# radiocosmology/draco

Hardware: AMD Instinct MI355X
Metric: m-modes/sec through MModeTransform+DirtyMapMaker (128-feed, 256-freq) (higher is better)
Workload: dtype f64 accumulate; B stored complex128; FFT complex64 (as the reference); 1 GPU; cfg3: 128-feed (379 stacked baselines), 256 freq per GPU (256 in the job), 1024 RA, lmax=mmax=512: MModeTransform.process + DirtyMapMaker.process through the task classes (131328 (m,f) solves + alm2map to nside=256 IQUV maps per GPU and day); parallelism=freq-sharded x1, weak scaling (no collective in the timed region)

## Files before the change

### draco_amd/csrc/sht.hip

```cpp
#include "sht_common.h"
#include "sht_legendre.h"
#include "sht_rings.h"

namespace {

int get_geom(dmm_ctx* ctx, int nside, int lmax, int mmax, ShtGeom* out) {
  const int64_t key = ((int64_t)nside << 40) | ((int64_t)lmax << 20) | (int64_t)mmax;
  auto it = ctx->sht.find(key);
  const int nring = 4 * nside - 1;
  const size_t nd = (size_t)3 * nring + (mmax + 1);
  const size_t bytes = nd * sizeof(double) + (size_t)nring * sizeof(int64_t) + (size_t)nring * sizeof(int);
  const size_t coef_ofs = (bytes + 63) / 64 * 64;
  const size_t coef_rows = (size_t)coef_row0(mmax + 1, lmax);
  int blue_rmax = 0;
  std::vector<int64_t> bf_off(1, 0);
  int64_t bf_total = 0;
  for (int ir = 1; ir < nside && blue_len(ir) <= kMaxBlue; ++ir) {
    bf_off.push_back(bf_total);
    bf_total += blue_len(ir);
    blue_rmax = ir;
  }
  const size_t bfo_ofs = coef_ofs + coef_rows * sizeof(Coef);
  const size_t bf_ofs = (bfo_ofs + bf_off.size() * sizeof(int64_t) + 63) / 64 * 64;
  const size_t phase_ofs = (bf_ofs + (size_t)bf_total * sizeof(double2) + 63) / 64 * 64;
  int tw_len = kMaxBlue;
  while (tw_len < 4 * nside) tw_len <<= 1;
  const size_t tw_ofs = phase_ofs + (size_t)nring * (mmax + 1) * sizeof(double2);
  const size_t chirp_ofs = tw_ofs + (size_t)(tw_len / 2) * sizeof(double2);
  const size_t total = chirp_ofs + (size_t)2 * blue_rmax * (blue_rmax + 1) * sizeof(double2);
  if (it == ctx->sht.end()) {
    std::vector<unsigned char> h(bytes);
    double* z = reinterpret_cast<double*>(h.data());
    double* sth = z + nring;
    double* phi0 = sth + nring;
    double* lfac = phi0 + nring;
    int64_t* start = reinterpret_cast<int64_t*>(lfac + (mmax + 1));
    int* nphi = reinterpret_cast<int*>(start + nring);
    const int64_t npix = 12LL * nside * nside, ncap = 2LL * nside * (nside - 1);
    for (int k = 0; k < nring; ++k) {
      const int64_t ir = k + 1;
      if (ir < nside) {
        z[k] = 1.0 - (double)(ir * ir) / (3.0 * nside * (double)nside);
        nphi[k] = (int)(4 * ir);
        phi0[k] = M_PI / (4.0 * ir);
        start[k] = 2 * ir * (ir - 1);
      } else if (ir <= 3LL * nside) {
        z[k] = (2.0 * nside - ir) * 2.0 / (3.0 * nside);
        nphi[k] = 4 * nside;
        phi0[k] = ((ir - nside + 1) & 1) * M_PI / (4.0 * nside);
        start[k] = ncap + (ir - nside) * 4LL * nside;
      } else {
        const int64_t ip = 4LL * nside - ir;
        z[k] = -(1.0 - (double)(ip * ip) / (3.0 * nside * (double)nside));
        nphi[k] = (int)(4 * ip);
        phi0[k] = M_PI / (4.0 * ip);
        start[k] = npix - 2 * ip * (ip + 1);
      }
      sth[k] = sqrt((1.0 - z[k]) * (1.0 + z[k]));
    }
    double acc = 0.5 * (log2(1.0) - log2(4.0 * M_PI));
    lfac[0] = acc;
    double prod = 0.0;
    for (int m = 1; m <= mmax; ++m) {
      prod += log2((2.0 * m - 1.0) / (2.0 * m));
      lfac[m] = 0.5 * (log2(2.0 * m + 1.0) - log2(4.0 * M_PI) + prod);
    }
    void* d = nullptr;
    DMM_HIP(hipMalloc(&d, total));
    unsigned char* db = static_cast<unsigned char*>(d);
    hipError_t e = hipMemcpy(d, h.data(), bytes, hipMemcpyHostToDevice);
    if (e == hipSuccess) e = hipMemcpy(db + bfo_ofs, bf_off.data(), bf_off.size() * sizeof(int64_t), hipMemcpyHostToDevice);
    if (e == hipSuccess) {
      hipLaunchKernelGGL(k_fill_coef, dim3(mmax + 1), dim3(256), 0, ctx->stream, reinterpret_cast<Coef*>(db + coef_ofs), lmax);
      e = hipGetLastError();
    }
    if (e == hipSuccess && blue_rmax > 0) {
      const int Mmax = blue_len(blue_rmax);
      const size_t lds = ((size_t)Mmax + 1 + Mmax / 2) * sizeof(double2);
      e = hipFuncSetAttribute((const void*)k_build_bfilt, hipFuncAttributeMaxDynamicSharedMemorySize, (int)lds);
      if (e == hipSuccess) {
        hipLaunchKernelGGL(k_build_bfilt, dim3(blue_rmax), dim3(kFftThreads), lds, ctx->stream,
                           reinterpret_cast<double2*>(db + bf_ofs), reinterpret_cast<const int64_t*>(db + bfo_ofs));
        e = hipGetLastError();
      }
    }
    if (e == hipSuccess) {
      hipLaunchKernelGGL(k_fill_ring_tables, dim3(nring + 1 + blue_rmax), dim3(256), 0, ctx->stream,
                         reinterpret_cast<const double*>(db) + 2 * (size_t)nring , nring, mmax,
                         reinterpret_cast<double2*>(db + phase_ofs), reinterpret_cast<double2*>(db + tw_ofs), tw_len,
                         reinterpret_cast<double2*>(db + chirp_ofs));
      e = hipGetLastError();
    }
    if (e != hipSuccess) {
      (void)hipFree(d);
      return dmm_set_error((int)e, "sht geometry upload: %s", hipGetErrorString(e));
    }
    it = ctx->sht.emplace(key, d).first;
  }
  ShtGeom g;
  g.nside = nside;
  g.lmax = lmax;
  g.mmax = mmax;
  g.nring = nring;
  g.block = it->second;
  g.z = reinterpret_cast<double*>(g.block);
  g.sth = g.z + nring;
  g.phi0 = g.sth + nring;
  g.lfac = g.phi0 + nring;
  g.start = reinterpret_cast<int64_t*>(g.lfac + (mmax + 1));
  g.nphi = reinterpret_cast<int*>(g.start + nring);
  unsigned char* gb = static_cast<unsigned char*>(g.block);
  g.coef = reinterpret_cast<double*>(gb + coef_ofs);
  g.bf_off = reinterpret_cast<int64_t*>(gb + bfo_ofs);
  g.bfilt = reinterpret_cast<double2*>(gb + bf_ofs);
  g.blue_rmax = blue_rmax;
  g.phase = reinterpret_cast<double2*>(gb + phase_ofs);
  g.tw = reinterpret_cast<double2*>(gb + tw_ofs);
  g.tw_len = tw_len;
  g.chirp = reinterpret_cast<double2*>(gb + chirp_ofs);
  *out = g;
  return DMM_OK;
}

int check_args(const char* who, dmm_ctx* ctx, const void* a, const void* b, int nfreq, int npol, int lmax, int mmax,
               int nside) {
  DMM_REQUIRE(ctx && a && b, "%s: NULL argument", who);
  DMM_REQUIRE(nfreq >= 1 && lmax >= 0 && mmax >= 0 && mmax <= lmax, "%s: bad sizes nfreq=%d lmax=%d mmax=%d", who, nfreq, lmax, mmax);
  DMM_REQUIRE(npol == 1 || npol == 4, "%s: npol must be 1 or 4 (got %d)", who, npol);
  DMM_REQUIRE(nside >= 1 && (nside & (nside - 1)) == 0 && nside <= 8192, "%s: nside must be a power of two (got %d)", who, nside);
  return DMM_OK;
}

size_t chunk_freqs(int nfreq, int npol, int nring, int mmax) {
  const size_t grp = npol == 4 ? kSynF : 1;
  const size_t per_f = (size_t)npol * nring * (mmax + 1) * sizeof(double2);
  size_t nf = ((size_t)1 << 30) / per_f / grp * grp;
  if (nf < grp) nf = grp;
  if (nf > (size_t)nfreq) nf = nfreq;
  const size_t nchunk = ((size_t)nfreq + nf - 1) / nf;
  const size_t c = ((size_t)nfreq + nchunk - 1) / nchunk;
  return c < (size_t)nfreq ? (c + grp - 1) / grp * grp : c;
}

size_t coef_scratch_bytes(size_t nfc, int npol, int nring, int mmax) {
  const size_t nfs = npol == 4 ? (nfc + kSynF - 1) / kSynF * kSynF : nfc;
  return nfs * npol * nring * (size_t)(mmax + 1) * sizeof(double2);
}

struct ClassLaunch {
  RingClass rc;
  int nblock;
  int nphi_max;
  bool blue;
};

std::vector<ClassLaunch> ring_classes(const ShtGeom& g) {
  std::vector<ClassLaunch> out;
  ClassLaunch b;
  b.rc.belt = 1;
  b.rc.r_lo = b.rc.r_hi = 0;
  b.rc.M = 4 * g.nside;
  b.rc.logM = 0;
  while ((1 << b.rc.logM) < b.rc.M) ++b.rc.logM;
  b.nblock = 2 * g.nside + 1;
  b.nphi_max = 4 * g.nside;
  b.blue = false;
  out.push_back(b);
  for (int ir = 1; ir < g.nside;) {
    const int M = blue_len(ir);
    int hi = ir;
    while (hi + 1 < g.nside && blue_len(hi + 1) == M) ++hi;
    ClassLaunch c;
    c.rc.belt = 0;
    c.rc.r_lo = ir;
    c.rc.r_hi = hi;
    c.rc.M = M;
    c.rc.logM = 0;
    while ((1 << c.rc.logM) < M) ++c.rc.logM;
    c.nblock = 2 * (hi - ir + 1);
    c.nphi_max = 4 * hi;
    c.blue = true;
    out.push_back(c);
    ir = hi + 1;
  }
  return out;
}

size_t ring_fft_lds(const ShtGeom& g, const ClassLaunch& c, int nrow, int force_direct) {
  if (force_direct) return 0;
  if (c.blue && c.rc.r_hi > g.blue_rmax) return 0;
  const size_t lds = ((size_t)nrow * (c.rc.M + 1) + c.rc.M / 2 + (c.blue ? c.nphi_max : 0)) * sizeof(double2);
  return lds <= 160 * 1024 ? lds : 0;
}

size_t ring_synth_lds(const ShtGeom& g, const ClassLaunch& c, int nb, bool stage_all, int force_direct) {
  if (force_direct) return 0;
  if (c.blue && c.rc.r_hi > g.blue_rmax) return 0;
  const int nm = g.mmax + 1;
  const bool staged = stage_all || 4 * (c.blue ? c.rc.r_lo : g.nside) < nm;
  const size_t lds = ((size_t)nb * (c.rc.M + 1) + c.rc.M / 2 + (c.blue ? c.nphi_max : 0) + (staged ? (size_t)nb * 2 * nm : 0)) *
                     sizeof(double2);
  return lds <= 160 * 1024 ? lds : 0;
}

template <typename K>
int launch_ring(K kern, dim3 grid, int threads, size_t lds, hipStream_t st, const RingParams& rp, const RingClass& rc) {
  if (lds > 160 * 1024) return dmm_set_error(DMM_E_UNSUPPORTED, "SHT ring stage needs %zu bytes of LDS (nside too large)", lds);
  DMM_HIP(hipFuncSetAttribute((const void*)kern, hipFuncAttributeMaxDynamicSharedMemorySize, (int)lds));
  hipLaunchKernelGGL(kern, grid, dim3(threads), lds, st, rp, rc);
  DMM_HIP(hipGetLastError());
  return DMM_OK;
}

template <int NPOL>
int synth_chunk(dmm_ctx* ctx, const ShtGeom& g, const double2* alm, int n_m, int nf, double2* b, double* map) {
  LegParams lp;
  lp.g = g;
  lp.nf = nf;
  lp.npol = NPOL;
  lp.n_m = n_m;
  lp.alm = alm;
  lp.b = b;
  if (NPOL == 4 && !(ctx->opt_sht_variant & 8)) {
    const int npair = (g.nring + 1) / 2;
    const int nrc = (npair + kThreads - 1) / kThreads;
#ifdef LEG_STAMPS
    static unsigned long long* stamps_d = nullptr;
    const size_t nst = (size_t)(g.mmax + 1) * nrc * ((nf + 2 * kLegF - 1) / (2 * kLegF)) * 4 * 8;
    if (!stamps_d) (void)hipMalloc((void**)&stamps_d, 64 << 20);
    (void)hipMemsetAsync(stamps_d, 0, nst * 8, ctx->stream);
    lp.stamps = stamps_d;
#endif
    const int nx = g.mmax + 1;
    const int64_t col_bytes = (int64_t)4 * n_m * (g.lmax + 1) * (int64_t)sizeof(double2);
    const bool fits8 = 2 * kLegF * col_bytes < ((int64_t)1 << 32), fits4 = kLegF * col_bytes < ((int64_t)1 << 32);
    if ((ctx->opt_sht_variant & 64) || ctx->opt_sht_synth_form == 1 || !fits4) {
      const int nz = (nf + kLegF - 1) / kLegF;
      hipLaunchKernelGGL(k_leg_synth_mfma, dim3(nx, nrc, nz), dim3(kThreads), 0, ctx->stream, lp);
    } else if ((ctx->opt_sht_variant & 128) || !fits8) {
      const int nz = (nf + kLegF - 1) / kLegF;
      hipLaunchKernelGGL(k_leg_synth_mfma2<1>, dim3(nx, nrc, nz), dim3(kThreads), 0, ctx->stream, lp);
    } else {
      const int nz = (nf + 2 * kLegF - 1) / (2 * kLegF);
      hipLaunchKernelGGL(k_leg_synth_mfma2<2>, dim3(nx, nrc, nz), dim3(kThreads), 0, ctx->stream, lp);
    }
  } else
  switch (ctx->opt_sht_variant & 3) {
    case 1: hipLaunchKernelGGL((k_leg_synth<NPOL, 1, 1>), dim3(g.mmax + 1, nf), dim3(kThreads), 0, ctx->stream, lp); break;
    case 2: hipLaunchKernelGGL((k_leg_synth<NPOL, 2, 1>), dim3(g.mmax + 1, nf), dim3(kThreads), 0, ctx->stream, lp); break;
    case 3: hipLaunchKernelGGL((k_leg_synth<NPOL, 1, 6>), dim3(g.mmax + 1, nf), dim3(kThreads), 0, ctx->stream, lp); break;
    default: hipLaunchKernelGGL((k_leg_synth<NPOL, 2, 4>), dim3(g.mmax + 1, nf), dim3(kThreads), 0, ctx->stream, lp); break;
  }
  DMM_HIP(hipGetLastError());
  RingParams rp;
  rp.g = g;
  rp.nf = nf;
  rp.npol = NPOL;
  rp.b = b;
  rp.map = map;
  rp.map_ref = nullptr;
  rp.radix8 = (ctx->opt_sht_variant & 2048) ? 0 : 1;
  rp.npix = 12LL * g.nside * g.nside;
  rp.stage_all = 0;
  constexpr int KF = NPOL == 4 ? kSynF : 1;
  const dim3 per_ring((nf + KF - 1) / KF, NPOL == 4 ? 2 : 1);
  const int force_direct = ctx->opt_sht_variant & 4;
  for (const ClassLaunch& c : ring_classes(g)) {
    int nb = 0;
    size_t lds = 0;
    rp.stage_all = 0;
    for (int tier = 0; tier < 3 && nb == 0; ++tier)
      for (int b = KF; b >= 1 && nb == 0; b >>= 1) {
        const size_t l = ring_synth_lds(g, c, b, tier == 0, force_direct);
        if (l != 0 && l <= (tier < 2 ? (size_t)80 * 1024 : (size_t)160 * 1024)) nb = b, lds = l, rp.stage_all = tier == 0;
      }
    const dim3 grid(c.nblock, per_ring.x, per_ring.y);
    int rc;
    if (nb == 0) {
      rc = launch_ring(k_ring_synth<NPOL>, dim3(c.nblock, nf), kThreads, (size_t)NPOL * (g.mmax + 1) * sizeof(double2), ctx->stream, rp, c.rc);
    } else if (nb == 4) {
      rc = c.blue ? launch_ring(k_ring_synth_fft<NPOL, NPOL == 4 ? 4 : 1, true>, grid, kFftThreads, lds, ctx->stream, rp, c.rc)
                  : launch_ring(k_ring_synth_fft<NPOL, NPOL == 4 ? 4 : 1, false>, grid, kFftThreads, lds, ctx->stream, rp, c.rc);
    } else if (nb == 2) {
      rc = c.blue ? launch_ring(k_ring_synth_fft<NPOL, NPOL == 4 ? 2 : 1, true>, grid, kFftThreads, lds, ctx->stream, rp, c.rc)
                  : launch_ring(k_ring_synth_fft<NPOL, NPOL == 4 ? 2 : 1, false>, grid, kFftThreads, lds, ctx->stream, rp, c.rc);
    } else {
      rc = c.blue ? launch_ring(k_ring_synth_fft<NPOL, 1, true>, grid, kFftThreads, lds, ctx->stream, rp, c.rc)
                  : launch_ring(k_ring_synth_fft<NPOL, 1, false>, grid, kFftThreads, lds, ctx->stream, rp, c.rc);
    }
    if (rc) return rc;
  }
  return DMM_OK;
}

template <int NPOL>
int anal_chunk(dmm_ctx* ctx, const ShtGeom& g, const double* map, int n_m, int nf, double2* b, double2* alm, int accumulate,
               const double* map_ref = nullptr) {
  RingParams rp;
  rp.g = g;
  rp.nf = nf;
  rp.npol = NPOL;
  rp.b = b;
  rp.map = const_cast<double*>(map);
  rp.map_ref = map_ref;
  rp.radix8 = (ctx->opt_sht_variant & 2048) ? 0 : 1;
  rp.npix = 12LL * g.nside * g.nside;
  rp.stage_all = 0;
  constexpr int NROWS = NPOL == 4 ? 2 : 1;
  const int force_direct = ctx->opt_sht_variant & 4;
  for (const ClassLaunch& c : ring_classes(g)) {
    const size_t lds2 = ring_fft_lds(g, c, NROWS, force_direct), lds1 = ring_fft_lds(g, c, 1, force_direct);
    int rc;
    if (lds1 == 0) {
      rc = launch_ring(k_ring_anal<NPOL>, dim3(c.nblock, nf), kThreads, (size_t)NPOL * c.nphi_max * sizeof(double), ctx->stream, rp, c.rc);
    } else if (NROWS == 2 && lds2 != 0 && lds2 <= 80 * 1024) {
      rc = c.blue ? launch_ring(k_ring_anal_fft<NPOL, NROWS, true>, dim3(c.nblock, nf), kFftThreads, lds2, ctx->stream, rp, c.rc)
                  : launch_ring(k_ring_anal_fft<NPOL, NROWS, false>, dim3(c.nblock, nf), kFftThreads, lds2, ctx->stream, rp, c.rc);
    } else {
      rc = c.blue ? launch_ring(k_ring_anal_fft<NPOL, 1, true>, dim3(c.nblock, nf, NROWS), kFftThreads, lds1, ctx->stream, rp, c.rc)
                  : launch_ring(k_ring_anal_fft<NPOL, 1, false>, dim3(c.nblock, nf, NROWS), kFftThreads, lds1, ctx->stream, rp, c.rc);
    }
    if (rc) return rc;
  }
  LegAnalParams lp;
  lp.g = g;
  lp.nf = nf;
  lp.npol = NPOL;
  lp.n_m = n_m;
  lp.b = b;
  lp.alm = alm;
  lp.accumulate = accumulate;
  lp.m_identity = (ctx->opt_sht_variant & 32) ? 1 : 0;
  if (NPOL == 4 && !(ctx->opt_sht_variant & 8)) {
    if (ctx->opt_sht_variant & 16)
      hipLaunchKernelGGL((k_leg_anal_mfma<kAnThreads, 1>), dim3(g.mmax + 1, (nf + kLegF - 1) / kLegF), dim3(kAnThreads), 0, ctx->stream, lp);
    else
      hipLaunchKernelGGL((k_leg_anal_mfma<256, 1>), dim3(g.mmax + 1, (nf + kLegF - 1) / kLegF), dim3(256), 0, ctx->stream, lp);
    DMM_HIP(hipGetLastError());
    return DMM_OK;
  }
  constexpr int NV = NPOL == 4 ? 8 : 2;
  const size_t lds2 = (size_t)(g.lmax + 1) * NV * sizeof(double) + (size_t)2 * (kThreads / 64) * kAnalBatch * NV * sizeof(double);
  DMM_HIP(hipFuncSetAttribute((const void*)k_leg_anal<NPOL>, hipFuncAttributeMaxDynamicSharedMemorySize, (int)lds2));
  hipLaunchKernelGGL(k_leg_anal<NPOL>, dim3(g.mmax + 1, nf), dim3(kThreads), lds2, ctx->stream, lp);
  DMM_HIP(hipGetLastError());
  return DMM_OK;
}

}

extern "C" {

int dmm_alm2map(dmm_ctx* ctx, const void* alm, int nfreq, int npol, int lmax, int mmax, int nside, double* map) {
  int rc = check_args("dmm_alm2map", ctx, alm, map, nfreq, npol, lmax, mmax, nside);
  if (rc) return rc;
  DMM_HIP(hipSetDevice(ctx->device));
  ShtGeom g;
  rc = get_geom(ctx, nside, lmax, mmax, &g);
  if (rc) return rc;
  const size_t nfc = chunk_freqs(nfreq, npol, g.nring, mmax);
  void* scratch = nullptr;
  rc = dmm_get_scratch(ctx, coef_scratch_bytes(nfc, npol, g.nring, mmax), &scratch);
  if (rc) return rc;
  const int64_t npix = 12LL * nside * nside;
  const int n_m = mmax + 1;
  for (int f0 = 0; f0 < nfreq; f0 += (int)nfc) {
    const int nf = (int)((size_t)(nfreq - f0) < nfc ? (size_t)(nfreq - f0) : nfc);
    const double2* a = (const double2*)alm + (int64_t)f0 * npol * n_m * (lmax + 1);
    double* mp = map + (int64_t)f0 * npol * npix;
    rc = npol == 4 ? synth_chunk<4>(ctx, g, a, n_m, nf, (double2*)scratch, mp) : synth_chunk<1>(ctx, g, a, n_m, nf, (double2*)scratch, mp);
    if (rc) return rc;
  }
  return DMM_OK;
}

int dmm_map2alm(dmm_ctx* ctx, const double* map, int nfreq, int npol, int lmax, int mmax, int nside, int niter,
                void* alm) {
  int rc = check_args("dmm_map2alm", ctx, map, alm, nfreq, npol, lmax, mmax, nside);
  if (rc) return rc;
  DMM_REQUIRE(niter >= 0 && niter <= 64, "dmm_map2alm: niter=%d out of range", niter);
  if ((size_t)npol * 4 * nside * sizeof(double) > 150 * 1024)
    return dmm_set_error(DMM_E_UNSUPPORTED, "dmm_map2alm: nside=%d too large for the in-LDS ring stage", nside);
  DMM_HIP(hipSetDevice(ctx->device));
  ShtGeom g;
  rc = get_geom(ctx, nside, lmax, mmax, &g);
  if (rc) return rc;
  const int64_t npix = 12LL * nside * nside;
  size_t nfc = chunk_freqs(nfreq, npol, g.nring, mmax);
  const size_t b_bytes = coef_scratch_bytes(nfc, npol, g.nring, mmax);
  const size_t r_bytes = niter > 0 ? nfc * npol * (size_t)npix * sizeof(double) : 0;
  void* scratch = nullptr;
  rc = dmm_get_scratch(ctx, b_bytes + r_bytes, &scratch);
  if (rc) return rc;
  double2* b = (double2*)scratch;
  double* resid = (double*)((unsigned char*)scratch + b_bytes);
  const int n_m = mmax + 1;
  for (int f0 = 0; f0 < nfreq; f0 += (int)nfc) {
    const int nf = (int)((size_t)(nfreq - f0) < nfc ? (size_t)(nfreq - f0) : nfc);
    double2* a = (double2*)alm + (int64_t)f0 * npol * n_m * (lmax + 1);
    const double* mp = map + (int64_t)f0 * npol * npix;
    rc = npol == 4 ? anal_chunk<4>(ctx, g, mp, n_m, nf, b, a, 0) : anal_chunk<1>(ctx, g, mp, n_m, nf, b, a, 0);
    if (rc) return rc;
    for (int it = 0; it < niter; ++it) {
      rc = npol == 4 ? synth_chunk<4>(ctx, g, a, n_m, nf, b, resid) : synth_chunk<1>(ctx, g, a, n_m, nf, b, resid);
      if (rc) return rc;
      rc = npol == 4 ? anal_chunk<4>(ctx, g, resid, n_m, nf, b, a, 1, mp) : anal_chunk<1>(ctx, g, resid, n_m, nf, b, a, 1, mp);
      if (rc) return rc;
    }
  }
  return DMM_OK;
}

}
```

### draco_amd/csrc/sht_rings.h

```cpp
#pragma once
#include "sht_common.h"

namespace {

struct RingParams {
  ShtGeom g;
  int nf, npol;
  double2* b;
  double* map;
  int64_t npix;
  const double* map_ref;
  int radix8;
  int stage_all;
};

struct RingClass {
  int belt;
  int r_lo, r_hi;
  int M, logM;
};
constexpr int kMinBlue = 256, kMaxBlue = 4096;

__host__ __device__ __forceinline__ int blue_len(int ir) {
  int M = kMinBlue;
  while (M < 8 * ir - 1) M <<= 1;
  return M;
}

__device__ __forceinline__ int class_ring(const RingClass& rc, const ShtGeom& g, int i) {
  if (rc.belt) return g.nside - 1 + i;
  const int ir = rc.r_lo + (i >> 1);
  return (i & 1) ? g.nring - ir : ir - 1;
}

template <int NPOL>
__global__ __launch_bounds__(kThreads) void k_ring_synth(RingParams p, RingClass rc) {
  extern __shared__ __align__(16) unsigned char smem[];
  double2* c = reinterpret_cast<double2*>(smem);
  const int ring = class_ring(rc, p.g, blockIdx.x);
  const int f = blockIdx.y;
  const int nm = p.g.mmax + 1;
  const double phi0 = p.g.phi0[ring];
  const int nphi = p.g.nphi[ring];
  for (int idx = threadIdx.x; idx < NPOL * nm; idx += kThreads) {
    const int pol = idx / nm, m = idx - pol * nm;
    double2 v;
    if (NPOL == 1) {
      v = p.b[((int64_t)f * p.g.nring + ring) * nm + m];
    } else {
      const double* q = reinterpret_cast<const double*>(p.b) + syn4_at(f, m, ring, pol >> 1, p.g.nring, nm) + syn4_slot(pol);
      v = make_double2(q[0], q[2]);
    }
    double sn, cs;
    sincos((double)m * phi0, &sn, &cs);
    const double fac = m == 0 ? 1.0 : 2.0;
    c[idx] = make_double2(fac * (v.x * cs - v.y * sn), fac * (v.x * sn + v.y * cs));
  }
  __syncthreads();
  const int64_t base = p.g.start[ring];
  for (int j = threadIdx.x; j < nphi; j += kThreads) {
    double sn, cs;
    sincospi(2.0 * (double)j / (double)nphi, &sn, &cs);
    double pr = 1.0, pi_ = 0.0;
    double acc[NPOL];
#pragma unroll
    for (int q = 0; q < NPOL; ++q) acc[q] = 0.0;
    for (int m = 0; m < nm; ++m) {
#pragma unroll
      for (int q = 0; q < NPOL; ++q) {
        const double2 cm = c[q * nm + m];
        acc[q] = fma(cm.x, pr, fma(-cm.y, pi_, acc[q]));
      }
      const double nr = pr * cs - pi_ * sn;
      pi_ = fma(pr, sn, pi_ * cs);
      pr = nr;
    }
#pragma unroll
    for (int q = 0; q < NPOL; ++q) p.map[((int64_t)f * NPOL + q) * p.npix + base + j] = acc[q];
  }
}

constexpr int kFftThreads = 256;

struct RingLds {
  dmm_fft::C<double>* buf;
  dmm_fft::C<double>* tw;
  dmm_fft::C<double>* chirp;
};

template <int NROW, bool BLUE>
__device__ __forceinline__ RingLds ring_lds(unsigned char* smem, const ShtGeom& g, int N, int M) {
  RingLds l;
  l.buf = reinterpret_cast<dmm_fft::C<double>*>(smem);
  l.tw = l.buf + NROW * (M + 1);
  l.chirp = l.tw + (M >> 1);
  const int stride = g.tw_len / M;
  for (int k = threadIdx.x; k < (M >> 1); k += kFftThreads) {
    const double2 t = g.tw[k * stride];
    l.tw[k] = {t.x, t.y};
  }
  if (BLUE) {
    const int ir = N >> 2;
    const double2* src = g.chirp + (int64_t)2 * ir * (ir - 1);
    for (int k = threadIdx.x; k < N; k += kFftThreads) {
      const double2 t = src[k];
      l.chirp[k] = {t.x, t.y};
    }
  }
  return l;
}

__global__ void k_fill_ring_tables(const double* phi0, int nring, int mmax, double2* phase, double2* tw, int tw_len,
                                   double2* chirp) {
  const int b = blockIdx.x;
  if (b < nring) {
    const double p0 = phi0[b];
    for (int m = threadIdx.x; m <= mmax; m += blockDim.x) {
      double sn, cs;
      sincos((double)m * p0, &sn, &cs);
      phase[(int64_t)b * (mmax + 1) + m] = make_double2(cs, sn);
    }
  } else if (b == nring) {
    for (int k = threadIdx.x; k < tw_len / 2; k += blockDim.x) {
      double sn, cs;
      sincospi(-2.0 * (double)k / (double)tw_len, &sn, &cs);
      tw[k] = make_double2(cs, sn);
    }
  } else {
    const int ir = b - nring, N = 4 * ir;
    double2* dst = chirp + (int64_t)2 * ir * (ir - 1);
    for (int k = threadIdx.x; k < N; k += blockDim.x) {
      const int k2 = (int)(((int64_t)k * k) % (2 * (int64_t)N));
      double sn, cs;
      sincospi(-(double)k2 / (double)N, &sn, &cs);
      dst[k] = make_double2(cs, sn);
    }
  }
}

template <int NROW, bool BLUE>
__device__ __forceinline__ void ring_dft(const RingLds& l, const double2* bfilt, int M, int logM, bool radix8 = false) {
  const int P = M + 1;
  if (radix8) dmm_fft::fft_dif8<double, kFftThreads>(l.buf, l.tw, NROW, M, logM, P);
  else dmm_fft::fft_dif<double, kFftThreads>(l.buf, l.tw, NROW, M, logM, P);
  if (BLUE) {
    for (int idx = threadIdx.x; idx < NROW * M; idx += kFftThreads) {
      const int r = idx / M, k = idx - r * M;
      const double2 fk = bfilt[k];
      l.buf[r * P + k] = dmm_fft::cmul<double>(l.buf[r * P + k], {fk.x, fk.y});
    }
    __syncthreads();
    if (radix8) dmm_fft::fft_dit8<double, true, kFftThreads>(l.buf, l.tw, NROW, M, logM, P);
    else dmm_fft::fft_dit<double, true, kFftThreads>(l.buf, l.tw, NROW, M, logM, P);
  }
}

template <bool BLUE>
__device__ __forceinline__ dmm_fft::C<double> ring_dft_at(const RingLds& l, int r, int k, int M, int logM) {
  if (BLUE) return dmm_fft::cmul<double>(l.buf[r * (M + 1) + k], l.chirp[k]);
  return l.buf[r * (M + 1) + dmm_fft::bitrev(k, logM)];
}

template <int NPOL, int NB, bool BLUE>
__global__ __launch_bounds__(kFftThreads) void k_ring_synth_fft(RingParams p, RingClass rc) {
  using dmm_fft::C;
  constexpr int KF = NPOL == 4 ? kSynF : 1;
  static_assert(KF % NB == 0, "passes of NB transforms");
  extern __shared__ __align__(16) unsigned char smem[];
  const int ring = class_ring(rc, p.g, blockIdx.x), r = NPOL == 4 ? (int)blockIdx.z : 0;
  const int f0 = KF * blockIdx.y, nfb = min(KF, p.nf - f0);
  const int n = p.g.nphi[ring], M = rc.M, P = M + 1;
  const RingLds l = ring_lds<NB, BLUE>(smem, p.g, n, M);
  if (BLUE) __syncthreads();
  const int nm = p.g.mmax + 1;
  const double2* phase = p.g.phase + (int64_t)ring * nm;
  auto load = [&](int fi, int m, double2& va, double2& vb) {
    if (NPOL == 1) {
      va = p.b[((int64_t)(f0 + fi) * p.g.nring + ring) * nm + m];
    } else {
      const double* q = reinterpret_cast<const double*>(p.b) + syn4_at(f0 + fi, m, ring, r, p.g.nring, nm);
      const double2 re = *reinterpret_cast<const double2*>(q), im = *reinterpret_cast<const double2*>(q + 2);
      va = r == 0 ? make_double2(re.x, im.x) : make_double2(re.y, im.y);
      vb = r == 0 ? make_double2(re.y, im.y) : make_double2(re.x, im.x);
    }
  };
  const bool staged = p.stage_all || n < nm;
  C<double>* rot = l.chirp + (BLUE ? 4 * rc.r_hi : 0);
  const double2* bfilt = BLUE ? p.g.bfilt + p.g.bf_off[rc.belt ? 0 : rc.r_lo + ((int)blockIdx.x >> 1)] : nullptr;
  const int64_t base = p.g.start[ring];
  for (int fb = 0; fb < nfb; fb += NB) {
    if (fb > 0) __syncthreads();
    if (staged) {
      for (int q = threadIdx.x; q < NB * nm; q += kFftThreads) {
        const int m = q / NB, j = q - m * NB;
        C<double> a = {0.0, 0.0}, b = {0.0, 0.0};
        if (fb + j < nfb) {
          const double2 ph = phase[m];
          const double cs = ph.x, sn = ph.y;
          double2 va, vb;
          load(fb + j, m, va, vb);
          a = {va.x * cs - va.y * sn, va.x * sn + va.y * cs};
          if (NPOL == 4) b = {vb.x * cs - vb.y * sn, vb.x * sn + vb.y * cs};
          if (m == 0) a.y = b.y = 0.0;
        }
        rot[(j * 2 + 0) * nm + m] = a;
        rot[(j * 2 + 1) * nm + m] = b;
      }
      __syncthreads();
    }
    for (int k = threadIdx.x; k < M; k += kFftThreads) {
      double zr[NB], zi[NB];
#pragma unroll
      for (int j = 0; j < NB; ++j) zr[j] = zi[j] = 0.0;
      if (k < n && staged) {
        for (int m = k; m < nm; m += n) {
#pragma unroll
          for (int j = 0; j < NB; ++j) {
            const C<double> a = rot[(j * 2 + 0) * nm + m], b = rot[(j * 2 + 1) * nm + m];
            zr[j] += a.x - b.y;
            zi[j] += a.y + b.x;
          }
        }
        for (int m = (k == 0 ? n : n - k); m < nm; m += n) {
#pragma unroll
          for (int j = 0; j < NB; ++j) {
            const C<double> a = rot[(j * 2 + 0) * nm + m], b = rot[(j * 2 + 1) * nm + m];
            zr[j] += a.x + b.y;
            zi[j] += b.x - a.y;
          }
        }
      } else if (k < n) {
        for (int m = k; m < nm; m += n) {
          const double2 ph = phase[m];
          const double cs = ph.x, sn = ph.y;
#pragma unroll
          for (int j = 0; j < NB; ++j) {
            if (fb + j >= nfb) continue;
            double2 va, vb;
            load(fb + j, m, va, vb);
            double ar = va.x * cs - va.y * sn, ai = va.x * sn + va.y * cs;
            double br = 0.0, bi = 0.0;
            if (NPOL == 4) {
              br = vb.x * cs - vb.y * sn;
              bi = vb.x * sn + vb.y * cs;
            }
            if (m == 0) ai = bi = 0.0;
            zr[j] += ar - bi;
            zi[j] += ai + br;
          }
        }
        for (int m = (k == 0 ? n : n - k); m < nm; m += n) {
          const double2 ph = phase[m];
          const double cs = ph.x, sn = ph.y;
#pragma unroll
          for (int j = 0; j < NB; ++j) {
            if (fb + j >= nfb) continue;
            double2 va, vb;
            load(fb + j, m, va, vb);
            const double ar = va.x * cs - va.y * sn, ai = va.x * sn + va.y * cs;
            double br = 0.0, bi = 0.0;
            if (NPOL == 4) {
              br = vb.x * cs - vb.y * sn;
              bi = vb.x * sn + vb.y * cs;
            }
            zr[j] += ar + bi;
            zi[j] += br - ai;
          }
        }
      }
#pragma unroll
      for (int j = 0; j < NB; ++j) {
        C<double> v = {zr[j], -zi[j]};
        if (BLUE && k < n) v = dmm_fft::cmul<double>(v, l.chirp[k]);
        l.buf[j * P + k] = v;
      }
    }
    __syncthreads();
    ring_dft<NB, BLUE>(l, bfilt, M, rc.logM, p.radix8 != 0);
    for (int j = threadIdx.x; j < n; j += kFftThreads) {
#pragma unroll
      for (int jj = 0; jj < NB; ++jj) {
        if (fb + jj >= nfb) continue;
        const int64_t f = f0 + fb + jj;
        const C<double> y = ring_dft_at<BLUE>(l, jj, j, M, rc.logM);
        p.map[(f * NPOL + 2 * r) * p.npix + base + j] = y.x;
        if (NPOL == 4) p.map[(f * NPOL + 2 * r + 1) * p.npix + base + j] = -y.y;
      }
    }
  }
}

template <int NPOL>
__global__ __launch_bounds__(kThreads) void k_ring_anal(RingParams p, RingClass rc) {
  extern __shared__ __align__(16) unsigned char smem[];
  double* px = reinterpret_cast<double*>(smem);
  const int ring = class_ring(rc, p.g, blockIdx.x), f = blockIdx.y;
  const int nm = p.g.mmax + 1;
  const double phi0 = p.g.phi0[ring];
  const int nphi = p.g.nphi[ring];
  const int64_t base = p.g.start[ring];
  for (int idx = threadIdx.x; idx < NPOL * nphi; idx += kThreads) {
    const int pol = idx / nphi, j = idx - pol * nphi;
    const int64_t pi = ((int64_t)f * NPOL + pol) * p.npix + base + j;
    px[idx] = p.map_ref ? p.map_ref[pi] - p.map[pi] : p.map[pi];
  }
  __syncthreads();
  const double w = 4.0 * M_PI / (double)p.npix;
  for (int m = threadIdx.x; m < nm; m += kThreads) {
    double sn, cs;
    sincospi(-2.0 * (double)(m % nphi) / (double)nphi, &sn, &cs);
    double pr = 1.0, pi_ = 0.0;
    double are[NPOL], aim[NPOL];
#pragma unroll
    for (int q = 0; q < NPOL; ++q) are[q] = aim[q] = 0.0;
    for (int j = 0; j < nphi; ++j) {
#pragma unroll
      for (int q = 0; q < NPOL; ++q) {
        const double v = px[q * nphi + j];
        are[q] = fma(v, pr, are[q]);
        aim[q] = fma(v, pi_, aim[q]);
      }
      const double nr = pr * cs - pi_ * sn;
      pi_ = fma(pr, sn, pi_ * cs);
      pr = nr;
    }
    double s0, c0;
    sincos(-(double)m * phi0, &s0, &c0);
#pragma unroll
    for (int q = 0; q < NPOL; ++q)
      p.b[(((int64_t)f * NPOL + q) * p.g.nring + ring) * nm + m] =
          make_double2(w * (are[q] * c0 - aim[q] * s0), w * (are[q] * s0 + aim[q] * c0));
  }
}

template <int NPOL, int NROW, bool BLUE>
__global__ __launch_bounds__(kFftThreads) void k_ring_anal_fft(RingParams p, RingClass rc) {
  using dmm_fft::C;
  extern __shared__ __align__(16) unsigned char smem[];
  const int rb = blockIdx.z * NROW;
  const int ring = class_ring(rc, p.g, blockIdx.x), f = blockIdx.y;
  const int n = p.g.nphi[ring], M = rc.M, P = M + 1;
  const RingLds l = ring_lds<NROW, BLUE>(smem, p.g, n, M);
  if (BLUE) __syncthreads();
  const int64_t base = p.g.start[ring];
  for (int k = threadIdx.x; k < M; k += kFftThreads) {
#pragma unroll
    for (int r = 0; r < NROW; ++r) {
      C<double> v = {0.0, 0.0};
      if (k < n) {
        const int64_t p0 = ((int64_t)f * NPOL + (NPOL == 4 ? 2 * (r + rb) : 0)) * p.npix + base + k, p1 = p0 + p.npix;
        v.x = p.map_ref ? p.map_ref[p0] - p.map[p0] : p.map[p0];
        if (NPOL == 4) v.y = p.map_ref ? p.map_ref[p1] - p.map[p1] : p.map[p1];
        if (BLUE) v = dmm_fft::cmul<double>(v, l.chirp[k]);
      }
      l.buf[r * P + k] = v;
    }
  }
  __syncthreads();
  const double2* bfilt = BLUE ? p.g.bfilt + p.g.bf_off[rc.belt ? 0 : rc.r_lo + ((int)blockIdx.x >> 1)] : nullptr;
  ring_dft<NROW, BLUE>(l, bfilt, M, rc.logM, p.radix8 != 0);
  const int nm = p.g.mmax + 1;
  const double2* phase = p.g.phase + (int64_t)ring * nm;
  const double w = 4.0 * M_PI / (double)p.npix;
  for (int m = threadIdx.x; m < nm; m += kFftThreads) {
    const int k = m % n, k2 = (n - k) % n;
    const double2 ph = phase[m];
    const double c0 = ph.x, s0 = -ph.y;
#pragma unroll
    for (int r = 0; r < NROW; ++r) {
      const C<double> X = ring_dft_at<BLUE>(l, r, k, M, rc.logM), Y = ring_dft_at<BLUE>(l, r, k2, M, rc.logM);
      const double ar = 0.5 * (X.x + Y.x), ai = 0.5 * (X.y - Y.y);
      p.b[(((int64_t)f * NPOL + (NPOL == 4 ? 2 * (r + rb) : 0)) * p.g.nring + ring) * nm + m] =
          make_double2(w * (ar * c0 - ai * s0), w * (ar * s0 + ai * c0));
      if (NPOL == 4) {
        const double br = 0.5 * (X.y + Y.y), bi = -0.5 * (X.x - Y.x);
        p.b[(((int64_t)f * NPOL + 2 * (r + rb) + 1) * p.g.nring + ring) * nm + m] =
            make_double2(w * (br * c0 - bi * s0), w * (br * s0 + bi * c0));
      }
    }
  }
}

__global__ __launch_bounds__(kFftThreads) void k_build_bfilt(double2* table, const int64_t* bf_off) {
  using dmm_fft::C;
  extern __shared__ __align__(16) unsigned char smem[];
  const int ir = blockIdx.x + 1, N = 4 * ir, M = blue_len(ir), P = M + 1;
  int logM = 0;
  while ((1 << logM) < M) ++logM;
  C<double>* buf = reinterpret_cast<C<double>*>(smem);
  C<double>* tw = buf + P;
  for (int k = threadIdx.x; k < (M >> 1); k += kFftThreads) {
    double sn, cs;
    sincospi(-2.0 * (double)k / (double)M, &sn, &cs);
    tw[k] = {cs, sn};
  }
  for (int j = threadIdx.x; j < M; j += kFftThreads) {
    const int nn = j < N ? j : (j > M - N ? M - j : -1);
    C<double> v = {0.0, 0.0};
    if (nn >= 0) {
      const int k2 = (int)(((int64_t)nn * nn) % (2 * (int64_t)N));
      double sn, cs;
      sincospi((double)k2 / (double)N, &sn, &cs);
      v = {cs, sn};
    }
    buf[j] = v;
  }
  __syncthreads();
  dmm_fft::fft_dif<double, kFftThreads>(buf, tw, 1, M, logM, P);
  const double inv = 1.0 / (double)M;
  double2* out = table + bf_off[ir];
  for (int k = threadIdx.x; k < M; k += kFftThreads) out[k] = make_double2(buf[k].x * inv, buf[k].y * inv);
}

}
```

Measured before the change: 2059 m-modes/s.

## Add register-accumulating synth4 ring kernel that folds m-phases before FFT

```diff
diff --git a/draco_amd/csrc/sht.hip b/draco_amd/csrc/sht.hip
--- a/draco_amd/csrc/sht.hip
+++ b/draco_amd/csrc/sht.hip
@@ -193,14 +193,35 @@
   return lds <= 160 * 1024 ? lds : 0;
 }
 
-size_t ring_synth_lds(const ShtGeom& g, const ClassLaunch& c, int nb, bool stage_all, int force_direct) {
+size_t ring_synth_lds(const ShtGeom& g, const ClassLaunch& c, bool stage_all, int force_direct) {
   if (force_direct) return 0;
   if (c.blue && c.rc.r_hi > g.blue_rmax) return 0;
   const int nm = g.mmax + 1;
   const bool staged = stage_all || 4 * (c.blue ? c.rc.r_lo : g.nside) < nm;
-  const size_t lds = ((size_t)nb * (c.rc.M + 1) + c.rc.M / 2 + (c.blue ? c.nphi_max : 0) + (staged ? (size_t)nb * 2 * nm : 0)) *
-                     sizeof(double2);
+  const size_t lds = ((size_t)(c.rc.M + 1) + c.rc.M / 2 + (c.blue ? c.nphi_max : 0) + (staged ? (size_t)2 * nm : 0)) * sizeof(double2);
   return lds <= 160 * 1024 ? lds : 0;
+}
+
+struct Synth4Shape {
+  int nrow, kt, seg;
+  size_t lds;
+};
+Synth4Shape ring_synth4_shape(const ShtGeom& g, const ClassLaunch& c, int force_direct) {
+  Synth4Shape s = {1, 0, 0, 0};
+  if (force_direct || (c.blue && c.rc.r_hi > g.blue_rmax)) return s;
+  s.kt = c.nphi_max <= 4 * kFftThreads ? 4 : c.nphi_max <= 8 * kFftThreads ? 8 : 0;
+  if (s.kt == 0 || c.rc.M > 2 * s.kt * kFftThreads) return s;
+  const size_t cap = (size_t)80 * 1024 / sizeof(double2), nm = (size_t)g.mmax + 1;
+  const size_t fixed = (size_t)c.rc.M / 2 + (c.blue ? c.nphi_max : 0);
+  if (!c.blue && (size_t)kSynF * (c.rc.M + 1) + fixed <= cap) s.nrow = kSynF;
+  if (!c.blue && s.nrow == 1 && s.kt != 8) return s;
+  const size_t rows = (size_t)s.nrow * (c.rc.M + 1);
+  size_t seg = fixed < cap ? (cap - fixed) / (2 * kSynF) : 0;
+  seg = std::min(std::max(seg, rows / (2 * kSynF)), nm);
+  s.seg = (int)seg;
+  const size_t lds = (std::max(rows, 2 * kSynF * seg) + fixed) * sizeof(double2);
+  s.lds = lds <= 160 * 1024 ? lds : 0;
+  return s;
 }
 
 template <typename K>
@@ -262,31 +283,31 @@
   rp.radix8 = (ctx->opt_sht_variant & 2048) ? 0 : 1;
   rp.npix = 12LL * g.nside * g.nside;
   rp.stage_all = 0;
+  rp.seg = 0;
   constexpr int KF = NPOL == 4 ? kSynF : 1;
   const dim3 per_ring((nf + KF - 1) / KF, NPOL == 4 ? 2 : 1);
   const int force_direct = ctx->opt_sht_variant & 4;
   for (const ClassLaunch& c : ring_classes(g)) {
-    int nb = 0;
-    size_t lds = 0;
-    rp.stage_all = 0;
-    for (int tier = 0; tier < 3 && nb == 0; ++tier)
-      for (int b = KF; b >= 1 && nb == 0; b >>= 1) {
-        const size_t l = ring_synth_lds(g, c, b, tier == 0, force_direct);
-        if (l != 0 && l <= (tier < 2 ? (size_t)80 * 1024 : (size_t)160 * 1024)) nb = b, lds = l, rp.stage_all = tier == 0;
-      }
     const dim3 grid(c.nblock, per_ring.x, per_ring.y);
     int rc;
-    if (nb == 0) {
+    const Synth4Shape s4 = NPOL == 4 ? ring_synth4_shape(g, c, force_direct) : Synth4Shape{1, 0, 0, 0};
+    if (s4.lds != 0) {
+      rp.seg = s4.seg;
+      if (c.blue) rc = s4.kt == 4 ? launch_ring(k_ring_synth4<true, 1, 4>, grid, kFftThreads, s4.lds, ctx->stream, rp, c.rc)
+                                  : launch_ring(k_ring_synth4<true, 1, 8>, grid, kFftThreads, s4.lds, ctx->stream, rp, c.rc);
+      else rc = s4.nrow == kSynF ? launch_ring(k_ring_synth4<false, kSynF, 4>, grid, kFftThreads, s4.lds, ctx->stream, rp, c.rc)
+                                 : launch_ring(k_ring_synth4<false, 1, 8>, grid, kFftThreads, s4.lds, ctx->stream, rp, c.rc);
+      if (rc) return rc;
+      continue;
+    }
+    size_t lds = ring_synth_lds(g, c, true, force_direct);
+    rp.stage_all = lds != 0 && lds <= (size_t)80 * 1024;
+    if (!rp.stage_all) lds = ring_synth_lds(g, c, false, force_direct);
+    if (lds == 0) {
       rc = launch_ring(k_ring_synth<NPOL>, dim3(c.nblock, nf), kThreads, (size_t)NPOL * (g.mmax + 1) * sizeof(double2), ctx->stream, rp, c.rc);
-    } else if (nb == 4) {
-      rc = c.blue ? launch_ring(k_ring_synth_fft<NPOL, NPOL == 4 ? 4 : 1, true>, grid, kFftThreads, lds, ctx->stream, rp, c.rc)
-                  : launch_ring(k_ring_synth_fft<NPOL, NPOL == 4 ? 4 : 1, false>, grid, kFftThreads, lds, ctx->stream, rp, c.rc);
-    } else if (nb == 2) {
-      rc = c.blue ? launch_ring(k_ring_synth_fft<NPOL, NPOL == 4 ? 2 : 1, true>, grid, kFftThreads, lds, ctx->stream, rp, c.rc)
-                  : launch_ring(k_ring_synth_fft<NPOL, NPOL == 4 ? 2 : 1, false>, grid, kFftThreads, lds, ctx->stream, rp, c.rc);
     } else {
-      rc = c.blue ? launch_ring(k_ring_synth_fft<NPOL, 1, true>, grid, kFftThreads, lds, ctx->stream, rp, c.rc)
-                  : launch_ring(k_ring_synth_fft<NPOL, 1, false>, grid, kFftThreads, lds, ctx->stream, rp, c.rc);
+      rc = c.blue ? launch_ring(k_ring_synth_fft<NPOL, true>, grid, kFftThreads, lds, ctx->stream, rp, c.rc)
+                  : launch_ring(k_ring_synth_fft<NPOL, false>, grid, kFftThreads, lds, ctx->stream, rp, c.rc);
     }
     if (rc) return rc;
   }
@@ -306,6 +327,7 @@
   rp.radix8 = (ctx->opt_sht_variant & 2048) ? 0 : 1;
   rp.npix = 12LL * g.nside * g.nside;
   rp.stage_all = 0;
+  rp.seg = 0;
   constexpr int NROWS = NPOL == 4 ? 2 : 1;
   const int force_direct = ctx->opt_sht_variant & 4;
   for (const ClassLaunch& c : ring_classes(g)) {
diff --git a/draco_amd/csrc/sht_rings.h b/draco_amd/csrc/sht_rings.h
--- a/draco_amd/csrc/sht_rings.h
+++ b/draco_amd/csrc/sht_rings.h
@@ -12,6 +12,7 @@
   const double* map_ref;
   int radix8;
   int stage_all;
+  int seg;
 };
 
 struct RingClass {
@@ -89,10 +90,10 @@
 };
 
 template <int NROW, bool BLUE>
-__device__ __forceinline__ RingLds ring_lds(unsigned char* smem, const ShtGeom& g, int N, int M) {
+__device__ __forceinline__ RingLds ring_lds(unsigned char* smem, const ShtGeom& g, int N, int M, int nbuf = 0) {
   RingLds l;
   l.buf = reinterpret_cast<dmm_fft::C<double>*>(smem);
-  l.tw = l.buf + NROW * (M + 1);
+  l.tw = l.buf + (nbuf > 0 ? nbuf : NROW * (M + 1));
   l.chirp = l.tw + (M >> 1);
   const int stride = g.tw_len / M;
   for (int k = threadIdx.x; k < (M >> 1); k += kFftThreads) {
@@ -161,11 +162,11 @@
   return l.buf[r * (M + 1) + dmm_fft::bitrev(k, logM)];
 }
 
-template <int NPOL, int NB, bool BLUE>
+template <int NPOL, bool BLUE>
 __global__ __launch_bounds__(kFftThreads) void k_ring_synth_fft(RingParams p, RingClass rc) {
   using dmm_fft::C;
   constexpr int KF = NPOL == 4 ? kSynF : 1;
-  static_assert(KF % NB == 0, "passes of NB transforms");
+  constexpr int NB = 1;
   extern __shared__ __align__(16) unsigned char smem[];
   const int ring = class_ring(rc, p.g, blockIdx.x), r = NPOL == 4 ? (int)blockIdx.z : 0;
   const int f0 = KF * blockIdx.y, nfb = min(KF, p.nf - f0);
@@ -290,6 +291,134 @@
   }
 }
 
+template <bool BLUE, int NROW, int KT>
+__global__ __launch_bounds__(kFftThreads) void k_ring_synth4(RingParams p, RingClass rc) {
+  using dmm_fft::C;
+  static_assert(NROW == 1 || NROW == kSynF, "the group's transforms together or one at a time");
+  extern __shared__ __align__(16) unsigned char smem[];
+  const int ring = class_ring(rc, p.g, blockIdx.x), r = blockIdx.z;
+  const int f0 = kSynF * blockIdx.y, nfb = min(kSynF, p.nf - f0);
+  const int n = p.g.nphi[ring], M = rc.M, P = M + 1, S = p.seg;
+  const int nm = p.g.mmax + 1;
+  const RingLds l = ring_lds<NROW, false>(smem, p.g, n, M, max(NROW * P, 2 * kSynF * S));
+  if (BLUE) {
+    for (int k = threadIdx.x; k < n; k += kFftThreads) {
+      const int k2 = (int)(((int64_t)k * k) % (2 * (int64_t)n));
+      double sn, cs;
+      sincospi(-(double)k2 / (double)n, &sn, &cs);
+      l.chirp[k] = {cs, sn};
+    }
+  }
+  const double phi0 = p.g.phi0[ring];
+  const double* run = reinterpret_cast<const double*>(p.b) + syn4_at(f0, 0, ring, r, p.g.nring, nm);
+  C<double>* rot = l.buf;
+  double zr[KT][kSynF], zi[KT][kSynF];
+#pragma unroll
+  for (int i = 0; i < KT; ++i)
+#pragma unroll
+    for (int j = 0; j < kSynF; ++j) zr[i][j] = zi[i][j] = 0.0;
+  for (int m0 = 0; m0 < nm; m0 += S) {
+    const int m1 = min(m0 + S, nm);
+    if (m0 > 0) __syncthreads();
+    for (int q = threadIdx.x; q < kSynF * (m1 - m0); q += kFftThreads) {
+      const int mm = q / kSynF, j = q - mm * kSynF, m = m0 + mm;
+      C<double> a = {0.0, 0.0}, b = {0.0, 0.0};
+      if (j < nfb) {
+        double sn, cs;
+        sincos((double)m * phi0, &sn, &cs);
+        const double* qp = run + (int64_t)m * kSynRow + 4 * j;
+        const double2 re = *reinterpret_cast<const double2*>(qp), im = *reinterpret_cast<const double2*>(qp + 2);
+        const double2 va = r == 0 ? make_double2(re.x, im.x) : make_double2(re.y, im.y);
+        const double2 vb = r == 0 ? make_double2(re.y, im.y) : make_double2(re.x, im.x);
+        a = {va.x * cs - va.y * sn, va.x * sn + va.y * cs};
+        b = {vb.x * cs - vb.y * sn, vb.x * sn + vb.y * cs};
+        if (m == 0) a.y = b.y = 0.0;
+      }
+      rot[(j * 2 + 0) * S + mm] = a;
+      rot[(j * 2 + 1) * S + mm] = b;
+    }
+    __syncthreads();
+    const int m0n = m0 % n;
+#pragma unroll
+    for (int i = 0; i < KT; ++i) {
+      const int k = threadIdx.x + i * kFftThreads;
+      if (k >= n) continue;
+      int d = k - m0n;
+      for (int m = m0 + (d < 0 ? d + n : d); m < m1; m += n) {
+#pragma unroll
+        for (int j = 0; j < kSynF; ++j) {
+          const C<double> a = rot[(j * 2 + 0) * S + m - m0], b = rot[(j * 2 + 1) * S + m - m0];
+          zr[i][j] += a.x - b.y;
+          zi[i][j] += a.y + b.x;
+        }
+      }
+      d = (k == 0 ? 0 : n - k) - m0n;
+      int m = m0 + (d < 0 ? d + n : d);
+      if (m == 0) m = n;
+      for (; m < m1; m += n) {
+#pragma unroll
+        for (int j = 0; j < kSynF; ++j) {
+          const C<double> a = rot[(j * 2 + 0) * S + m - m0], b = rot[(j * 2 + 1) * S + m - m0];
+          zr[i][j] += a.x + b.y;
+          zi[i][j] += b.x - a.y;
+        }
+      }
+    }
+  }
+  double2 bf[BLUE ? 2 * KT : 1];
+  if (BLUE) {
+    const double2* bfilt = p.g.bfilt + p.g.bf_off[rc.r_lo + ((int)blockIdx.x >> 1)];
+#pragma unroll
+    for (int i = 0; i < 2 * KT; ++i) {
+      const int k = threadIdx.x + i * kFftThreads;
+      if (k < M) bf[i] = bfilt[k];
+    }
+  }
+  const int64_t base = p.g.start[ring];
+#pragma unroll
+  for (int j0 = 0; j0 < kSynF; j0 += NROW) {
+    if (j0 >= nfb) break;
+    __syncthreads();
+#pragma unroll
+    for (int i = 0; i < KT; ++i) {
+      const int k = threadIdx.x + i * kFftThreads;
+      if (k >= n) continue;
+#pragma unroll
+      for (int jr = 0; jr < NROW; ++jr) {
+        C<double> v = {zr[i][j0 + jr], -zi[i][j0 + jr]};
+        if (BLUE) v = dmm_fft::cmul<double>(v, l.chirp[k]);
+        l.buf[jr * P + k] = v;
+      }
+    }
+    for (int k = n + threadIdx.x; k < M; k += kFftThreads)
+#pragma unroll
+      for (int jr = 0; jr < NROW; ++jr) l.buf[jr * P + k] = {0.0, 0.0};
+    __syncthreads();
+    if (p.radix8) dmm_fft::fft_dif8<double, kFftThreads>(l.buf, l.tw, NROW, M, rc.logM, P);
+    else dmm_fft::fft_dif<double, kFftThreads>(l.buf, l.tw, NROW, M, rc.logM, P);
+    if (BLUE) {
+#pragma unroll
+      for (int i = 0; i < 2 * KT; ++i) {
+        const int k = threadIdx.x + i * kFftThreads;
+        if (k < M) l.buf[k] = dmm_fft::cmul<double>(l.buf[k], {bf[i].x, bf[i].y});
+      }
+      __syncthreads();
+      if (p.radix8) dmm_fft::fft_dit8<double, true, kFftThreads>(l.buf, l.tw, NROW, M, rc.logM, P);
+      else dmm_fft::fft_dit<double, true, kFftThreads>(l.buf, l.tw, NROW, M, rc.logM, P);
+    }
+    for (int jp = threadIdx.x; jp < n; jp += kFftThreads) {
+#pragma unroll
+      for (int jr = 0; jr < NROW; ++jr) {
+        if (j0 + jr >= nfb) continue;
+        const int64_t f = f0 + j0 + jr;
+        const C<double> y = ring_dft_at<BLUE>(l, jr, jp, M, rc.logM);
+        p.map[(f * 4 + 2 * r) * p.npix + base + jp] = y.x;
+        p.map[(f * 4 + 2 * r + 1) * p.npix + base + jp] = -y.y;
+      }
+    }
+  }
+}
+
 template <int NPOL>
 __global__ __launch_bounds__(kThreads) void k_ring_anal(RingParams p, RingClass rc) {
   extern __shared__ __align__(16) unsigned char smem[];
```

Result: no change. 2051 m-modes/s (median of 3 runs) (-0.4%).
